# dusk-network/plonk

Measured on NVIDIA H100. Metric: proofs/sec @ 2^16 gates, higher is better.
Workload: dtype u32 limbs (Fr 256-bit / Fp 384-bit Montgomery)

## Files before the change

plonk_b200/csrc/prover.cu:

```cuda
#include <algorithm>
#include <mutex>
#include <vector>

#include "compress.h"
#include "internal.cuh"
#include "host_field.h"
#include "plonk_algebra.cuh"
#include "transcript.h"

namespace pb {

static std::atomic<int> g_force_throughput{0};

PB_D Fr ldg_fr(const uint4* p, size_t i) {
  uint4 a = __ldg(p + 2 * i), b = __ldg(p + 2 * i + 1);
  Fr r;
  r.v[0] = a.x; r.v[1] = a.y; r.v[2] = a.z; r.v[3] = a.w;
  r.v[4] = b.x; r.v[5] = b.y; r.v[6] = b.z; r.v[7] = b.w;
  return r;
}
PB_D Fr ld_fr_plain(const uint4* p, size_t i) {
  uint4 a = p[2 * i], b = p[2 * i + 1];
  Fr r;
  r.v[0] = a.x; r.v[1] = a.y; r.v[2] = a.z; r.v[3] = a.w;
// ... 209 lines not shown
  if (tid == 255 && totals) {
    Fr tot = lds_pair(sh[cur][255]);
    stg_fr(totals, blockIdx.x, tot);
  }
}

template <bool MUL, bool REV>
__global__ void k_scan_fixup(uint4* out, size_t n, const uint4* block_prefix) {
  const size_t i = (size_t)blockIdx.x * blockDim.x + threadIdx.x;
  if (i >= n) return;
  const size_t blk = i / 2048;
  if (blk == 0) return;
  const size_t j = REV ? (n - 1 - i) : i;
  stg_fr(out, j, scan_op<MUL>(ld_fr_plain(block_prefix, blk), ld_fr_plain(out, j)));
}

struct QuotArgs {
  const uint4* w8;
  const uint4* key8;
  const uint4* linear8;
  const uint4* l1_8;
  uint4* out;
  size_t n8;
  Fr alpha, beta, gamma, alpha_sq;
  SepPowers<Fr> ch_range, ch_logic, ch_fixed, ch_var;
  Fr edwards_d;
  Fr vh_inv[8];
  int has_range, has_logic, has_fixed, has_var;
};

__device__ __noinline__ Fr fr_mul_outlined(Fr a, Fr b) { return a * b; }

struct Q {
  Fr v;
  PB_D Q() {}
  PB_D Q(const Fr& f) : v(f) {}
  static PB_D Q one() { return Q(Fr::one()); }
  static PB_D Q zero() { return Q(Fr::zero()); }
  friend PB_D Q operator+(const Q& x, const Q& y) { return Q(x.v + y.v); }
  friend PB_D Q operator-(const Q& x, const Q& y) { return Q(x.v - y.v); }
  friend PB_D Q operator*(const Q& x, const Q& y) { return Q(fr_mul_outlined(x.v, y.v)); }
  PB_D Q sqr() const { return Q(fr_mul_outlined(v, v)); }
  PB_D Q dbl() const { return Q(v.dbl()); }
};

PB_D void quotient_point(const QuotArgs& q, size_t ws, size_t i, size_t iw, size_t ki, size_t oi) {
  const size_t n8 = q.n8;
  WireVals<Q> v;
  const Q z = ldg_fr(q.w8, i), z_w = ldg_fr(q.w8, iw);
  v.a = ldg_fr(q.w8, ws + i); v.a_w = ldg_fr(q.w8, ws + iw);
  v.b = ldg_fr(q.w8, 2 * ws + i); v.b_w = ldg_fr(q.w8, 2 * ws + iw);
  v.c = ldg_fr(q.w8, 3 * ws + i);
  v.d = ldg_fr(q.w8, 4 * ws + i); v.d_w = ldg_fr(q.w8, 4 * ws + iw);
  const Q pi = ldg_fr(q.w8, 5 * ws + i);
#define KEY(k) ldg_fr(q.key8, (size_t)(k) * n8 + ki)
  const Q q_l = KEY(Q_L), q_r = KEY(Q_R), q_c = KEY(Q_C);
  Q t = (v.a * v.b * KEY(Q_M) + v.a * q_l + v.b * q_r + v.c * KEY(Q_O) + v.d * KEY(Q_F) + q_c) * KEY(Q_ARITH);
  if (q.has_range) t = t + widget_range(q.ch_range, v) * KEY(Q_RANGE);
  if (q.has_logic) t = t + widget_logic(q.ch_logic, q_c, v) * KEY(Q_LOGIC);
  if (q.has_fixed) t = t + widget_fixed(q.ch_fixed, Q(q.edwards_d), q_l, q_r, q_c, v) * KEY(Q_FIXED);
  if (q.has_var) t = t + widget_var(q.ch_var, Q(q.edwards_d), v) * KEY(Q_VAR);
  t = t + pi;
  const Q x = ldg_fr(q.linear8, ki);
  const Q alpha = q.alpha, beta = q.beta, gamma = q.gamma;
  const Q bx = beta * x;
  Q ident = perm_ident(v, bx, gamma) * z * alpha;
  Q copy = perm_copy3(v, beta, gamma, [&](int j) { return Q(KEY(S1 + j)); }) * (v.d + beta * KEY(S4) + gamma) * z_w * alpha;
#undef KEY
  Q l1 = Q(ldg_fr(q.l1_8, ki)) * Q(q.alpha_sq);
  t = t + ident - copy + (z - Q::one()) * l1;
  stg_fr(q.out, oi, (t * Q(q.vh_inv[ki & 7])).v);
}

__global__ void __launch_bounds__(128) k_quotient(QuotArgs q) {
  const size_t i = (size_t)blockIdx.x * blockDim.x + threadIdx.x;
  if (i >= q.n8) return;
  quotient_point(q, q.n8, i, (i + 8) & (q.n8 - 1), i, i);
}
template <int MINB>
__global__ void __launch_bounds__(128, MINB) k_quotient_4n(QuotArgs q) {
  const size_t i = (size_t)blockIdx.x * blockDim.x + threadIdx.x;
  const size_t n4 = q.n8 >> 1;
  if (i >= n4) return;
  quotient_point(q, n4, i, (i + 4) & (n4 - 1), 2 * i, i);
}
__global__ void __launch_bounds__(128) k_quotient_pts(QuotArgs q) {
  const size_t k = threadIdx.x;
  if (k >= 8) return;
  quotient_point(q, 16, k, k + 8, 1 + (q.n8 >> 3) * k, k);
}

__global__ void k_any_nonzero(const uint4* p, size_t lo, size_t hi, unsigned* flag) {
  size_t i = lo + (size_t)blockIdx.x * blockDim.x + threadIdx.x;
  if (i >= hi) return;
  uint4 a = p[2 * i], b = p[2 * i + 1];
  if (a.x | a.y | a.z | a.w | b.x | b.y | b.z | b.w) atomicOr(flag, 1u);
}

__global__ void k_split_quotient(const uint4* t, size_t n, size_t n8, size_t stride, Fr b12, Fr b13, Fr b14, uint4* out) {
  size_t i = (size_t)blockIdx.x * blockDim.x + threadIdx.x;
  if (i >= stride) return;
  const unsigned k = blockIdx.y;
  Fr v = Fr::zero();
  if (k < 3) {
    if (i < n) v = ld_fr_plain(t, (size_t)k * n + i);
    if (i == n) v = (k == 0) ? b12 : (k == 1 ? b13 : b14);
    if (i == 0 && k == 1) v = v - b12;
    if (i == 0 && k == 2) v = v - b13;
  } else {
    if (3 * n + i < n8) v = ld_fr_plain(t, 3 * n + i);
    if (i == 0) v = v - b14;
  }
  stg_fr(out, (size_t)k * stride + i, v);
}

PB_D void cta_poly_eval(const uint4* poly, unsigned len, const Fr& x, uint4* out_slot) {
  __shared__ uint4 sh[256][2];
  const int tid = threadIdx.x;
  const size_t base = ((size_t)blockIdx.x * 256 + tid) * 8;
  Fr acc = Fr::zero();
  if (base < len) {
#pragma unroll
    for (int k = 7; k >= 0; k--) {
      const Fr c = (base + k < len) ? ld_fr_plain(poly, base + k) : Fr::zero();
      acc = acc * x + c;
    }
  }
  sh[tid][0] = make_uint4(acc.v[0], acc.v[1], acc.v[2], acc.v[3]);
  sh[tid][1] = make_uint4(acc.v[4], acc.v[5], acc.v[6], acc.v[7]);
  Fr pw = x.sqr().sqr().sqr();
  __syncthreads();
  for (int d = 1; d < 256; d <<= 1) {
    if ((tid & (2 * d - 1)) == 0) {
      const Fr v = lds_pair(sh[tid]) + lds_pair(sh[tid + d]) * pw;
      sh[tid][0] = make_uint4(v.v[0], v.v[1], v.v[2], v.v[3]);
      sh[tid][1] = make_uint4(v.v[4], v.v[5], v.v[6], v.v[7]);
      pw = pw.sqr();
    }
    __syncthreads();
  }
  if (tid == 0) stg_fr(out_slot, 0, lds_pair(sh[0]));
}

struct EvalJobs {
  const uint4* poly[16];
  unsigned len[16];
  Fr point[16];
  int njobs;
};
__global__ void __launch_bounds__(256) k_poly_eval(EvalJobs jobs, uint4* partial, unsigned nblocks) {
  const int j = blockIdx.y;
  cta_poly_eval(jobs.poly[j], jobs.len[j], jobs.point[j], partial + 2 * ((size_t)j * nblocks + blockIdx.x));
}
struct EvalRows {
  const uint4* base;
  size_t row_stride;
  unsigned len;
  Fr point[16];
};
__global__ void __launch_bounds__(256) k_poly_eval_rows(EvalRows jobs, uint4* partial, unsigned nblocks) {
  cta_poly_eval(jobs.base + 2 * (size_t)blockIdx.z * jobs.row_stride, jobs.len, jobs.point[blockIdx.y],
                partial + 2 * (((size_t)blockIdx.z * gridDim.y + blockIdx.y) * nblocks + blockIdx.x));
}
struct EvalPoints {
  Fr p[16];
};
__global__ void k_sum_rows(const uint4* partial, unsigned nblocks, EvalPoints pts, int npts, uint4* out) {
  const int j = blockIdx.x;
  if (threadIdx.x != 0) return;
  Fr step = pts.p[j % npts];
#pragma unroll 1
  for (int k = 0; k < 11; k++) step = step.sqr();
  Fr acc = Fr::zero();
#pragma unroll 1
  for (unsigned b = nblocks; b-- > 0;) acc = acc * step + ld_fr_plain(partial, (size_t)j * nblocks + b);
  stg_fr(out, j, acc);
}

struct Quot4nFix {
  Fr c;
  Fr g4n;
  Fr hinv8[8];
  Fr w8inv_pow[8];
};
__global__ void k_quot4n_fix(const uint4* tx, const uint4* ux, uint4* tcoef, size_t n4, Quot4nFix f, unsigned* flag) {
  const int j = threadIdx.x;
  if (j >= 8) return;
  Fr acc = Fr::zero();
  for (int k = 0; k < 8; k++) {
    const Fr e = (ld_fr_plain(tx, k) - ld_fr_plain(ux, k)) * f.c;
    acc = acc + e * f.w8inv_pow[(j * k) & 7];
  }
  const Fr t_hi = acc * f.hinv8[j];
  if (j == 7) {
    if (!t_hi.is_zero()) atomicOr(flag, 1u);
    return;
  }
  stg_fr(tcoef, j, ld_fr_plain(tcoef, j) - f.g4n * t_hi);
  stg_fr(tcoef, n4 + j, t_hi);
}

struct LinArgs {
  const uint4* poly[24];
  unsigned len[24];
  Fr coef[24];
  int nterms;
};
__global__ void k_lincomb(LinArgs a, size_t n, uint4* out) {
  size_t i = (size_t)blockIdx.x * blockDim.x + threadIdx.x;
  if (i >= n) return;
  Fr acc = Fr::zero();
  for (int k = 0; k < a.nterms; k++)
    if (i < a.len[k]) acc = acc + ld_fr_plain(a.poly[k], i) * a.coef[k];
  stg_fr(out, i, acc);
}

__global__ void k_mul_pointwise(const uint4* a, const uint4* b, size_t n, uint4* out) {
  size_t i = (size_t)blockIdx.x * blockDim.x + threadIdx.x;
  if (i < n) stg_fr(out, i, ld_fr_plain(a, i) * ld_fr_plain(b, i));
}
__global__ void k_sub_one(uint4* p, size_t n) {
  size_t i = (size_t)blockIdx.x * blockDim.x + threadIdx.x;
  if (i < n) stg_fr(p, i, ld_fr_plain(p, i) - Fr::one());
}
struct Period8 {
  Fr c[8];
};
__global__ void k_scale_period8(uint4* p, size_t n, Period8 c) {
  size_t i = (size_t)blockIdx.x * blockDim.x + threadIdx.x;
  if (i < n) stg_fr(p, i, ld_fr_plain(p, i) * c.c[i & 7]);
}

struct Quot4nConsts {
  Fr xs[16];
  Quot4nFix fix;
};

}

using pbh::HFr;

struct pb200_prover {
  std::vector<uint8_t> label;
  size_t constraints = 0, n = 0, n8 = 0;
  int log_n = 0;
  pb200_srs* srs = nullptr;
  pb200_srs* srs_lag = nullptr;
  uint32_t* d_wires = nullptr;
  uint4* d_polys = nullptr;
  uint4* d_key8 = nullptr;
  uint4* d_linear8 = nullptr;
  uint4* d_l1_8 = nullptr;
  uint4* d_sigma = nullptr;
  HFr vh_inv[8];
  pb::Fr edwards_d;
  pb::Quot4nConsts q4;
  int has_widget[4] = {0, 0, 0, 0};
  uint8_t comm[pb::N_POLY][48];
  size_t n_witnesses = 0;
  unsigned long long* d_labels = nullptr;
  size_t n_labels = 0;
  mutable std::mutex ws_mu;
  mutable std::vector<pb::Arena> ws_free;
  mutable std::vector<char*> ws_all;
  size_t ws_bytes = 0;
  mutable std::atomic<int> active{0};
};

namespace pb {

static Fr to_dev(const HFr& x) {
  Fr r;
  memcpy(r.v, x.v, 32);
  return r;
}
static HFr to_host(const Fr& x) {
  HFr r;
  memcpy(r.v, x.v, 32);
  return r;
}

template <bool MUL, bool REV>
static int fr_scan(const uint4* in, size_t n, uint4* out, cudaStream_t st, Arena* ar) {
  const unsigned nblk = div_up(n, 2048);
  uint4 *tot = nullptr, *tot_scan = nullptr;
  ScratchScope scope(ar, st);
  PB_ALLOC(scope, tot, (size_t)nblk * 32);
  PB_ALLOC(scope, tot_scan, (size_t)nblk * 32);
  PB_LAUNCH((k_scan_local<MUL, REV>), nblk, 256, 0, st, in, n, out, tot);
  if (nblk > 1) {
    PB_TRY((fr_scan<MUL, false>((const uint4*)tot, (size_t)nblk, tot_scan, st, ar)));
    PB_LAUNCH((k_scan_fixup<MUL, REV>), div_up(n, 256), 256, 0, st, out, n, (const uint4*)tot_scan);
  }
  PB_CUDA(cudaGetLastError());
  return 0;
}
static size_t fr_scan_bytes(size_t n) {
  const size_t nblk = div_up(n, 2048);
  return 2 * Arena::round_up(nblk * 32) + (nblk > 1 ? fr_scan_bytes(nblk) : 0);
}

enum ProofBuf { kWv, kZp, kNum, kDen, kW8, kQuot, kTcoef, kTq, kAgg, kPw, kScratch, kEvals, kPartial, kFlag, kProofBufs };
static void proof_buffers(size_t n, size_t bytes[kProofBufs]) {
  const size_t stride = n + 8;
  bytes[kWv] = 5 * n * 32;
  bytes[kZp] = 6 * stride * 32;
  bytes[kNum] = bytes[kDen] = n * 32;
  bytes[kW8] = 6 * 8 * n * 32;
  bytes[kQuot] = bytes[kTcoef] = 8 * n * 32;
  bytes[kTq] = 4 * stride * 32;
  bytes[kAgg] = bytes[kPw] = bytes[kScratch] = 2 * stride * 32;
  bytes[kEvals] = 16 * 32;
  bytes[kPartial] = (size_t)16 * div_up(stride, 2048) * 32;
  bytes[kFlag] = 4;
}

static void compress_affine(const uint64_t* raw, uint8_t out[48]) { pbh::g1_compress_raw(raw, out); }

void prover_free(pb200_prover* P);

struct PoolBlock {
  void* p = nullptr;
  cudaStream_t st;
  explicit PoolBlock(cudaStream_t s) : st(s) {}
  ~PoolBlock() {
    if (p) cudaFreeAsync(p, st);
  }
  cudaError_t alloc(size_t bytes) { return cudaMallocAsync(&p, bytes, st); }
  PoolBlock(const PoolBlock&) = delete;
  PoolBlock& operator=(const PoolBlock&) = delete;
};

struct LoadedProverKey {
  const uint8_t* poly[N_POLY];
  size_t poly_len[N_POLY];
  uint8_t comm[N_POLY][48];
};

static int prover_build(pb200_prover* P, const uint8_t* label, size_t label_len, size_t constraints, const uint64_t* selectors,
                        const uint32_t* wires, size_t n_witnesses, const uint8_t* srs_raw, size_t n_srs, cudaStream_t st,
                        const LoadedProverKey* loaded = nullptr, const pbz::CompressedDescription* comp = nullptr) {
  P->label.assign(label, label + label_len);
  P->constraints = constraints;
  P->n_witnesses = n_witnesses;
  size_t n_trim = 1;
  while (n_trim < constraints + 6) n_trim <<= 1;
  size_t keep = n_trim + 6;
  if (keep + 1 > n_srs) return fail(PB200_ERR_DEGREE_TOO_LARGE, "public parameters too small for this circuit (TruncatedDegreeTooLarge)");
  size_t n = 1;
  int log_n = 0;
  while (n < constraints) {
    n <<= 1;
    log_n++;
  }
  P->n = n;
  P->n8 = 8 * n;
  P->log_n = log_n;
  if (log_n + 3 >= 32) return fail(PB200_ERR_INVALID_DOMAIN, "quotient domain too large");
  PB_TRY(srs_upload(srs_raw, keep + 1, &P->srs, 0));
  {
    static const bool lagrange_env = [] {
      const char* e = getenv("PB200_LAGRANGE");
      return !e || atoi(e) != 0;
    }();
    if (lagrange_env && n >= 2 && keep + 1 >= n + 2) {
      uint4* comb = nullptr;
      PB_CUDA(cudaMalloc((void**)&comb, (n + 4) * 96));
      const uint4* mono = srs_points(P->srs);
      int rc = lagrange_key_dev(mono, log_n, comb, st);
      const size_t idx[4] = {0, 1, n, n + 1};
      cudaError_t e = cudaSuccess;
      for (int k = 0; k < 4 && e == cudaSuccess; k++)
        e = cudaMemcpyAsync(comb + 6 * (n + k), mono + 6 * idx[k], 96, cudaMemcpyDeviceToDevice, st);
      if (e == cudaSuccess) e = cudaStreamSynchronize(st);
      int lag_c = std::min(12, msm_window_for(n + 4));
      if (const char* env = getenv("PB200_LAG_C")) lag_c = atoi(env);
      if (lag_c < 2 || lag_c > 20) lag_c = 0;
      if (rc == 0 && e == cudaSuccess) rc = srs_from_device(comb, n + 4, &P->srs_lag, lag_c);
      cudaFree(comb);
      PB_TRY(rc);
      PB_CUDA(e);
    }
  }
  const size_t n8 = P->n8;
  PB_CUDA(cudaMalloc((void**)&P->d_wires, 4 * constraints * 4));
  PB_CUDA(cudaMalloc((void**)&P->d_polys, (size_t)N_POLY * n * 32));
  PB_CUDA(cudaMalloc((void**)&P->d_key8, (size_t)N_POLY * n8 * 32));
  PB_CUDA(cudaMalloc((void**)&P->d_linear8, n8 * 32));
  PB_CUDA(cudaMalloc((void**)&P->d_l1_8, n8 * 32));
  PB_CUDA(cudaMalloc((void**)&P->d_sigma, 4 * n * 32));
  PB_CUDA(cudaMemcpyAsync(P->d_wires, wires, 4 * constraints * 4, cudaMemcpyHostToDevice, st));

  if (loaded) {
    for (size_t g = 0; g < constraints; g++)
      for (int k = 0; k < 4; k++)
        if (wires[(size_t)k * constraints + g] >= n_witnesses) return fail(PB200_ERR_INVALID_ARG, "wire index out of range");
    PB_CUDA(cudaMemsetAsync(P->d_polys, 0, (size_t)N_POLY * n * 32, st));
    for (int k = 0; k < N_POLY; k++)
      if (loaded->poly_len[k])
        PB_CUDA(cudaMemcpyAsync(P->d_polys + 2 * (size_t)k * n, loaded->poly[k], loaded->poly_len[k] * 32, cudaMemcpyHostToDevice, st));
    PoolBlock flag_block(st);
    PB_CUDA(flag_block.alloc(4));
    unsigned* d_flag = (unsigned*)flag_block.p;
    PB_CUDA(cudaMemsetAsync(d_flag, 0, 4, st));
    PB_LAUNCH(k_fr_from_canonical, div_up((size_t)N_POLY * n, 256), 256, 0, st, P->d_polys, (size_t)N_POLY * n, d_flag);
    unsigned h_flag = 0;
    PB_CUDA(cudaMemcpyAsync(&h_flag, d_flag, 4, cudaMemcpyDeviceToHost, st));
    PB_CUDA(cudaStreamSynchronize(st));
    if (h_flag) return fail(PB200_ERR_POINT_MALFORMED, "InvalidData: a prover-key scalar is not canonical");
    memcpy(P->comm, loaded->comm, sizeof P->comm);
    const int widget_sel[4] = {Q_RANGE, Q_LOGIC, Q_FIXED, Q_VAR};
    for (int w = 0; w < 4; w++) P->has_widget[w] = (P->comm[widget_sel[w]][0] & 0x40) ? 0 : 1;
  } else {
    PoolBlock cols_block(st);
    PB_CUDA(cols_block.alloc((size_t)N_POLY * n * 32));
    uint4* cols = (uint4*)cols_block.p;
    if (!comp) {
      PB_CUDA(cudaMemsetAsync(cols, 0, (size_t)N_POLY * n * 32, st));
      PB_CUDA(cudaMemcpy2DAsync(cols, n * 32, selectors, constraints * 32, constraints * 32, 11, cudaMemcpyHostToDevice, st));
    } else {
      const size_t n_sc = comp->scalars.size() / 32, n_pw = comp->polynomials.size();
      PoolBlock tab_block(st);
      PB_CUDA(tab_block.alloc(Arena::round_up(n_sc * 32) + Arena::round_up(n_pw * 4) + constraints * 4 + 4));
      uint4* d_sc = (uint4*)tab_block.p;
      uint32_t* d_pw = (uint32_t*)((char*)tab_block.p + Arena::round_up(n_sc * 32));
      uint32_t* d_gp = d_pw + Arena::round_up(n_pw * 4) / 4;
      unsigned* d_flag = d_gp + constraints;
      PB_CUDA(cudaMemcpyAsync(d_sc, comp->scalars.data(), n_sc * 32, cudaMemcpyHostToDevice, st));
      PB_CUDA(cudaMemcpyAsync(d_pw, comp->polynomials.data(), n_pw * 4, cudaMemcpyHostToDevice, st));
      PB_CUDA(cudaMemcpyAsync(d_gp, comp->gate_poly.data(), constraints * 4, cudaMemcpyHostToDevice, st));
      PB_CUDA(cudaMemsetAsync(d_flag, 0, 4, st));
      PB_LAUNCH(k_fr_from_canonical, div_up(n_sc, 256), 256, 0, st, d_sc, n_sc, d_flag);
      PB_LAUNCH(k_expand_selectors, dim3(div_up(n, 256), pbz::kSelectors), 256, 0, st, (const uint4*)d_sc, (const uint32_t*)d_pw,
                (const uint32_t*)d_gp, constraints, n, cols);
      unsigned h_flag = 0;
      PB_CUDA(cudaMemcpyAsync(&h_flag, d_flag, 4, cudaMemcpyDeviceToHost, st));
      PB_CUDA(cudaStreamSynchronize(st));
      if (h_flag) return fail(PB200_ERR_SCALAR_MALFORMED, "BlsScalarMalformed: a compressed circuit's scalar is not canonical");
      PB_CUDA(cudaMalloc((void**)&P->d_labels, comp->labels.size() * 8));
      PB_CUDA(cudaMemcpy(P->d_labels, comp->labels.data(), comp->labels.size() * 8, cudaMemcpyHostToDevice));
      P->n_labels = comp->labels.size();
    }
    {
      const size_t n_ids = comp ? comp->labels.size() : n_witnesses;
      std::vector<std::vector<uint64_t>> wmap(n_ids);
      for (size_t g = 0; g < constraints; g++)
        for (int k = 0; k < 4; k++) {
          const uint32_t w = wires[(size_t)k * constraints + g];
          if (w >= n_ids) {
            return fail(PB200_ERR_INVALID_ARG, "wire index out of range");
          }
          wmap[w].push_back(((uint64_t)k << 40) | g);
        }
      std::vector<unsigned long long> sig(4 * n);
      for (int k = 0; k < 4; k++)
        for (size_t i = 0; i < n; i++) sig[(size_t)k * n + i] = ((uint64_t)k << 40) | i;
      for (auto& lst : wmap)
        for (size_t i = 0; i < lst.size(); i++) {
          const uint64_t cur = lst[i], nxt = lst[(i + 1) % lst.size()];
          sig[(size_t)(cur >> 40) * n + (cur & 0xffffffffffull)] = nxt;
        }
      PoolBlock sig_block(st);
      PB_CUDA(sig_block.alloc(4 * n * 8));
      unsigned long long* d_sig = (unsigned long long*)sig_block.p;
      PB_CUDA(cudaMemcpyAsync(d_sig, sig.data(), 4 * n * 8, cudaMemcpyHostToDevice, st));
      const uint4* w_half = nullptr;
      PB_TRY(get_twiddles(log_n, false, st, &w_half));
      PB_LAUNCH(k_sigma_lagrange, div_up(4 * n, 256), 256, 0, st, d_sig, n, w_half, cols + 2 * (size_t)S1 * n);
      PB_CUDA(cudaStreamSynchronize(st));
    }
    PB_TRY(ntt_run((const uint64_t*)cols, n, (uint64_t*)P->d_polys, log_n, 1, 0, N_POLY, n, n, st, nullptr));
    {
      std::vector<uint64_t> aff((size_t)N_POLY * 12);
      PB_TRY(msm_run(P->srs, 0, (const uint64_t*)P->d_polys, n, N_POLY, n, kMsmLatency, aff.data(), st, nullptr));
      for (int k = 0; k < N_POLY; k++) compress_affine(aff.data() + 12 * k, P->comm[k]);
      const int widget_sel[4] = {Q_RANGE, Q_LOGIC, Q_FIXED, Q_VAR};
      for (int w = 0; w < 4; w++) P->has_widget[w] = (P->comm[widget_sel[w]][0] & 0x40) ? 0 : 1;
    }
  }
  PB_TRY(ntt_run((const uint64_t*)P->d_polys, n, (uint64_t*)P->d_key8, log_n + 3, 0, 1, N_POLY, n, n8, st, nullptr));
  {
    HFr lin[2] = {HFr::zero(), HFr::one()};
    PoolBlock lin_block(st);
    PB_CUDA(lin_block.alloc(64));
    uint4* d_lin = (uint4*)lin_block.p;
    PB_CUDA(cudaMemcpyAsync(d_lin, lin, 64, cudaMemcpyHostToDevice, st));
    PB_TRY(ntt_run((const uint64_t*)d_lin, 2, (uint64_t*)P->d_linear8, log_n + 3, 0, 1, 1, 2, n8, st, nullptr));
    PB_CUDA(cudaStreamSynchronize(st));
  }
  {
    const HFr g = to_host(ntt_coset_gen(false)), w8n = to_host(ntt_group_gen(log_n + 3, false));
    HFr point = g.pow_u64(n), step = w8n.pow_u64(n);
    const HFr psi = to_host(ntt_size_inv(log_n + 3)) * HFr::from_u64(8);
    Period8 c;
    for (int i = 0; i < 8; i++) {
      const HFr vh = point - HFr::one();
      P->vh_inv[i] = vh.inv();
      c.c[i] = to_dev(vh * psi);
      point = point * step;
    }
    PB_CUDA(cudaMemcpyAsync(P->d_l1_8, P->d_linear8, n8 * 32, cudaMemcpyDeviceToDevice, st));
    PB_LAUNCH(k_sub_one, div_up(n8, 256), 256, 0, st, P->d_l1_8, n8);
    PB_LAUNCH(k_batch_div, div_up(div_up(n8, 8), 128), 128, 0, st, (const uint4*)nullptr, (const uint4*)P->d_l1_8, n8, P->d_l1_8);
    PB_LAUNCH(k_scale_period8, div_up(n8, 256), 256, 0, st, P->d_l1_8, n8, c);
  }
  {
    P->edwards_d = to_dev(pbh::edwards_d());
    const HFr g = to_host(ntt_coset_gen(false)), w8n = to_host(ntt_group_gen(log_n + 3, false));
    const HFr h = g * w8n, w8r = w8n.pow_u64(n), wn = to_host(ntt_group_gen(log_n, false)), g4n = g.pow_u64(4 * n);
    HFr xs[16];
    xs[0] = h;
    for (int k = 1; k < 8; k++) xs[k] = xs[k - 1] * w8r;
    for (int k = 0; k < 8; k++) xs[8 + k] = xs[k] * wn;
    for (int k = 0; k < 16; k++) P->q4.xs[k] = to_dev(xs[k]);
    P->q4.fix.c = to_dev((g4n.dbl().neg()).inv());
    P->q4.fix.g4n = to_dev(g4n);
    const HFr h_inv = h.inv(), w8i = w8r.inv();
    HFr hj = HFr::from_u64(8).inv(), wp = HFr::one();
    for (int j = 0; j < 8; j++) {
      P->q4.fix.hinv8[j] = to_dev(hj);
      P->q4.fix.w8inv_pow[j] = to_dev(wp);
      hj = hj * h_inv;
      wp = wp * w8i;
    }
  }
  PB_TRY(ntt_run((const uint64_t*)(P->d_polys + 2 * (size_t)S1 * n), n, (uint64_t*)P->d_sigma, log_n, 0, 0, 4, n, n, st, nullptr));
  PB_CUDA(cudaGetLastError());
  PB_CUDA(cudaStreamSynchronize(st));
  {
    const size_t stride = n + 8;
    size_t call = std::max((size_t)6 * n8 * 32, fr_scan_bytes(stride));
    call = std::max(call, msm_workspace_bytes(P->srs, std::min(stride, srs_len(P->srs)), 4));
    if (P->srs_lag) call = std::max(call, msm_workspace_bytes(P->srs_lag, n + 4, 4));
    size_t bytes[kProofBufs];
    proof_buffers(n, bytes);
    P->ws_bytes = call;
    for (size_t b : bytes) P->ws_bytes += Arena::round_up(b);
    P->ws_bytes += Arena::round_up(P->n_labels * 32);
  }
  return 0;
}

int prover_new(const uint8_t* label, size_t label_len, size_t constraints, const uint64_t* selectors,
               const uint32_t* wires, size_t n_witnesses, const uint8_t* srs_raw, size_t n_srs, pb200_prover** out) {
  if (constraints == 0) return fail(PB200_ERR_INVALID_ARG, "empty circuit");
  pb200_prover* P = new pb200_prover();
  const int rc = prover_build(P, label, label_len, constraints, selectors, wires, n_witnesses, srs_raw, n_srs, thread_stream());
  if (rc != 0) {
    prover_free(P);
    return rc;
  }
  *out = P;
  return 0;
}

int prover_from_compressed(const uint8_t* label, size_t label_len, const uint8_t* bytes, size_t len, const uint8_t* srs_raw,
                           size_t n_srs, pb200_prover** out) {
  pbz::CompressedDescription d;
  PB_TRY(pbz::decode(bytes, len, n_srs, &d));
  if (d.gates() == 0) return fail(PB200_ERR_INVALID_ARG, "empty circuit");
  pb200_prover* P = new pb200_prover();
  const int rc = prover_build(P, label, label_len, d.gates(), nullptr, d.wires.data(), (size_t)d.witnesses, srs_raw, n_srs,
                              thread_stream(), nullptr, &d);
  if (rc != 0) {
    prover_free(P);
    return rc;
  }
  *out = P;
  return 0;
}

int prover_from_bytes(const uint8_t* bytes, size_t len, const uint32_t* wires, size_t n_witnesses, pb200_prover** out) {
  auto be64 = [](const uint8_t* p) {
    uint64_t v = 0;
    for (int i = 0; i < 8; i++) v = (v << 8) | p[i];
    return v;
  };
  auto le64 = [](const uint8_t* p) {
    uint64_t v = 0;
    for (int i = 7; i >= 0; i--) v = (v << 8) | p[i];
    return v;
  };
  const int short_rc = PB200_ERR_INVALID_ARG, bad_rc = PB200_ERR_POINT_MALFORMED;
  if (len < 48) return fail(short_rc, "NotEnoughBytes: serialized prover shorter than its header");
  const uint64_t label_len = be64(bytes), pk_len = be64(bytes + 8), ck_len = be64(bytes + 16), vk_len = be64(bytes + 24),
                 size = be64(bytes + 32), constraints = be64(bytes + 40);
  const uint8_t* p = bytes + 48;
  size_t left = len - 48;
  if (label_len > left || pk_len > left - label_len || ck_len > left - label_len - pk_len || vk_len > left - label_len - pk_len - ck_len)
    return fail(short_rc, "NotEnoughBytes: serialized prover shorter than its sections");
  size_t pow2 = 1;
  while (pow2 < constraints) pow2 <<= 1;
  if (constraints == 0 || pow2 != size) return fail(bad_rc, "InvalidData: size is not the next power of two of the constraint count");
  const uint8_t* label = p;
  const uint8_t* pk = label + label_len;
  const uint8_t* ck = pk + pk_len;
  const uint8_t* vk = ck + ck_len;
  LoadedProverKey key;
  {
    size_t off = 0;
    auto need = [&](size_t k) { return k <= pk_len - off; };
    if (pk_len < 16) return fail(short_rc, "NotEnoughBytes: prover key");
    const uint64_t n = le64(pk), eval_size = le64(pk + 8);
    off = 16;
    if (n != size) return fail(bad_rc, "InvalidData: prover key domain differs from the prover's size");
    if (eval_size != 8 * n * 32 + 172) return fail(bad_rc, "InvalidData: evaluations are not over the 8n domain");
    for (int i = 0; i < N_POLY; i++) {
      if (!need(8)) return fail(short_rc, "NotEnoughBytes: prover key polynomial header");
      const uint64_t cnt = le64(pk + off);
      off += 8;
      if (cnt > n) return fail(bad_rc, "InvalidData: polynomial longer than the domain");
      if (!need(cnt * 32)) return fail(short_rc, "NotEnoughBytes: prover key polynomial");
      key.poly[kKeyFileOrder[i]] = pk + off;
      key.poly_len[kKeyFileOrder[i]] = (size_t)cnt;
      off += cnt * 32;
      if (!need(eval_size)) return fail(short_rc, "NotEnoughBytes: prover key evaluations");
      off += eval_size;
    }
    if (!need(2 * eval_size)) return fail(short_rc, "NotEnoughBytes: linear / vanishing evaluations");
  }
  if (vk_len < 8 + 15 * 48) return fail(short_rc, "NotEnoughBytes: verifier key");
  for (int i = 0; i < N_POLY; i++) memcpy(key.comm[kKeyFileOrder[i]], vk + 8 + 48 * i, 48);
  size_t n_pts = 0;
  PB_TRY(raw_commit_key_parse(ck, ck_len, 1, &n_pts, nullptr));
  std::vector<uint8_t> raw(n_pts * 96);
  PB_TRY(raw_commit_key_parse(ck, ck_len, 1, &n_pts, raw.data()));
  PB_TRY(g1_check_raw(raw.data(), n_pts));
  pb200_prover* P = new pb200_prover();
  const int rc = prover_build(P, label, label_len, constraints, nullptr, wires, n_witnesses, raw.data(), n_pts, thread_stream(), &key);
  if (rc != 0) {
    prover_free(P);
    return rc;
  }
  *out = P;
  return 0;
}

struct KeyStreamer {
  static constexpr size_t kChunk = (size_t)8 << 20;
  cudaStream_t st;
  uint4* d_buf[2] = {nullptr, nullptr};
  uint8_t* h_buf[2] = {nullptr, nullptr};
  cudaEvent_t ev[2] = {nullptr, nullptr};
  struct Pending {
    uint8_t* dst = nullptr;
    size_t count = 0;
    bool points = false;
  } pend[2];
  unsigned issued = 0;

  explicit KeyStreamer(cudaStream_t s) : st(s) {}
  ~KeyStreamer() {
    for (int b = 0; b < 2; b++) {
      if (pend[b].count) cudaEventSynchronize(ev[b]);
      if (d_buf[b]) cudaFreeAsync(d_buf[b], st);
      if (ev[b]) cudaEventDestroy(ev[b]);
    }
  }
  KeyStreamer(const KeyStreamer&) = delete;
  KeyStreamer& operator=(const KeyStreamer&) = delete;

  int init() {
    for (int b = 0; b < 2; b++) {
      PB_CUDA(cudaMallocAsync((void**)&d_buf[b], kChunk, st));
      h_buf[b] = (uint8_t*)pinned_scratch(kChunk, b);
      if (!h_buf[b]) return fail(PB200_ERR_CUDA, "pinned staging buffer allocation failed");
      PB_CUDA(cudaEventCreateWithFlags(&ev[b], cudaEventBlockingSync | cudaEventDisableTiming));
// ... 190 lines not shown
  PB_TRY(get_twiddles(log_n, false, st, &w_half));

  Arena arena;
  {
    std::lock_guard<std::mutex> lk(P->ws_mu);
    if (!P->ws_free.empty()) {
      arena = P->ws_free.back();
      P->ws_free.pop_back();
    }
  }
  if (!arena.base) {
    char* mem = nullptr;
    PB_CUDA(cudaMalloc((void**)&mem, P->ws_bytes));
    arena.base = mem;
    arena.size = P->ws_bytes;
    std::lock_guard<std::mutex> lk(P->ws_mu);
    P->ws_all.push_back(mem);
  }
  arena.off = 0;
  struct Release {
    const pb200_prover* P;
    Arena* a;
    cudaStream_t st;
    ~Release() {
      stream_wait(st);
      a->off = 0;
      std::lock_guard<std::mutex> lk(P->ws_mu);
      P->ws_free.push_back(*a);
    }
  } release{P, &arena, st};
  Arena* ar = &arena;
  ScratchScope scope(ar, st);
  const unsigned eval_blocks = div_up(stride, 2048);
  size_t bytes[kProofBufs];
  void* kept[kProofBufs];
  proof_buffers(n, bytes);
  for (int i = 0; i < kProofBufs; i++) PB_ALLOC(scope, kept[i], bytes[i]);
  uint4 *wv = (uint4*)kept[kWv], *zp = (uint4*)kept[kZp], *num = (uint4*)kept[kNum], *den = (uint4*)kept[kDen], *w8 = (uint4*)kept[kW8],
        *quot = (uint4*)kept[kQuot], *tcoef = (uint4*)kept[kTcoef], *tq = (uint4*)kept[kTq], *agg = (uint4*)kept[kAgg],
        *pw = (uint4*)kept[kPw], *scratch = (uint4*)kept[kScratch], *evals_d = (uint4*)kept[kEvals], *partial = (uint4*)kept[kPartial];
  unsigned* flag = (unsigned*)kept[kFlag];
  uint4 *wp = zp + 2 * stride, *pi_dense = wv + 2 * 4 * n;

  uint64_t aff[4 * 12];
  uint8_t c48[N_COMM][48];
  Challenges ch;

  if (P->d_labels) {
    uint4* dense = nullptr;
    PB_ALLOC(scope, dense, P->n_labels * 32);
    PB_LAUNCH(k_gather_witnesses, div_up(P->n_labels, 256), 256, 0, st, (const uint4*)d_wit, (const unsigned long long*)P->d_labels,
              P->n_labels, dense);
    d_wit = (const uint64_t*)dense;
  }

  PB_LAUNCH(k_gather_wires, dim3(div_up(n, 256), 4), 256, 0, st, (const uint4*)d_wit, (const uint32_t*)P->d_wires, P->constraints, n, wv);
  if (n_pi) {
    PB_CUDA(cudaMemsetAsync(pi_dense, 0, n * 32, st));
    for (size_t i = 0; i < n_pi; i++)
      PB_CUDA(cudaMemcpyAsync(pi_dense + 2 * pi_idx[i], PIV + i, 32, cudaMemcpyHostToDevice, st));
  }
  PB_CUDA(cudaMemsetAsync(zp, 0, 6 * stride * 32, st));
  PB_TRY(ntt_run((const uint64_t*)wv, n, (uint64_t*)wp, log_n, 1, 0, n_pi ? 5 : 4, n, stride, st, ar));
  {
    BlindArgs ba;
    ba.nb = 2;
    ba.npoly = 4;
    for (int p = 0; p < 4; p++)
      for (int i = 0; i < 2; i++) ba.b[p][i] = to_dev(BL[2 * p + i]);
    PB_LAUNCH(k_blind, 1, 32, 0, st, wp, stride, n, ba);
  }
  if (P->srs_lag) {
    uint4* sc = w8;
    PB_CUDA(cudaMemcpy2DAsync(sc, stride * 32, wv, n * 32, n * 32, 4, cudaMemcpyDeviceToDevice, st));
    BlindArgs ba;
    ba.nb = 2;
    ba.npoly = 4;
    for (int p = 0; p < 4; p++)
      for (int i = 0; i < 2; i++) ba.b[p][i] = to_dev(BL[2 * p + i]);
    PB_LAUNCH(k_lagrange_tail, 1, 32, 0, st, sc, stride, n, ba);
    PB_TRY(msm_run(P->srs_lag, 0, (const uint64_t*)sc, n + 4, 4, stride, MsmShape{true, busy()}, aff, st, ar));
  } else {
    PB_TRY(msm_run(P->srs, 0, (const uint64_t*)wp, n + 2, 4, stride, dense_shape(), aff, st, ar));
  }
  for (int k = 0; k < 4; k++) compress_affine(aff + 12 * k, c48[C_A + k]);

  pbh::challenge_beta_gamma(tr, c48[0], ch);
  const HFr beta = ch.beta, gamma = ch.gamma;
  PB_LAUNCH(k_perm_terms, div_up(n, 128), 128, 0, st, (const uint4*)wv, (const uint4*)P->d_sigma, w_half, n, to_dev(beta), to_dev(gamma), num, den);
  PB_LAUNCH(k_batch_div, div_up(div_up(n, 8), 128), 128, 0, st, (const uint4*)num, (const uint4*)den, n, num);
  PB_TRY((fr_scan<true, false>(num, n, den, st, ar)));
  PB_TRY(ntt_run((const uint64_t*)den, n, (uint64_t*)zp, log_n, 1, 0, 1, n, stride, st, ar));
  {
    BlindArgs ba;
    ba.nb = 3;
    ba.npoly = 1;
    for (int i = 0; i < 3; i++) ba.b[0][i] = to_dev(BL[8 + i]);
    PB_LAUNCH(k_blind, 1, 32, 0, st, zp, stride, n, ba);
  }
  PB_TRY(msm_run(P->srs, 0, (const uint64_t*)zp, n + 3, 1, stride, dense_shape(), aff, st, ar));
  compress_affine(aff, c48[C_Z]);

  pbh::challenge_alpha(tr, c48[0], ch);
  const HFr alpha = ch.alpha;
  static const bool quot4n_env = [] {
    const char* e = getenv("PB200_QUOT4N");
    return !e || atoi(e) != 0;
  }();
  const bool quot4n = quot4n_env && n >= 16;
  const size_t n4 = 4 * n;
  size_t t_len = n8;
  QuotArgs q;
  {
    q.w8 = w8; q.key8 = P->d_key8; q.linear8 = P->d_linear8; q.l1_8 = P->d_l1_8; q.out = quot; q.n8 = n8;
    q.alpha = to_dev(alpha); q.beta = to_dev(beta); q.gamma = to_dev(gamma); q.alpha_sq = to_dev(alpha.sqr());
    auto powers = [](const HFr& c) {
      const SepPowers<HFr> h = sep_powers(c);
      SepPowers<Fr> s;
      s.ch = to_dev(h.ch); s.k = to_dev(h.k); s.k2 = to_dev(h.k2); s.k3 = to_dev(h.k3); s.k4 = to_dev(h.k4);
      return s;
    };
    q.ch_range = powers(ch.range); q.ch_logic = powers(ch.logic); q.ch_fixed = powers(ch.fixed); q.ch_var = powers(ch.var);
    q.edwards_d = P->edwards_d;
    for (int i = 0; i < 8; i++) q.vh_inv[i] = to_dev(P->vh_inv[i]);
    q.has_range = P->has_widget[0]; q.has_logic = P->has_widget[1]; q.has_fixed = P->has_widget[2]; q.has_var = P->has_widget[3];
  }
  unsigned char* stage = (unsigned char*)pinned_scratch(1024, 1);
  if (!stage) return fail(PB200_ERR_CUDA, "pinned staging buffer");
  volatile unsigned& h_flag = *(volatile unsigned*)(stage + 512);
  if (!quot4n) {
    PB_TRY(ntt_run((const uint64_t*)zp, n + 3, (uint64_t*)w8, log_n + 3, 0, 1, n_pi ? 6 : 5, stride, n8, st, ar));
    if (!n_pi) PB_CUDA(cudaMemsetAsync(w8 + 2 * 5 * n8, 0, n8 * 32, st));
    PB_LAUNCH(k_quotient, div_up(n8, 128), 128, 0, st, q);
    PB_TRY(ntt_run((const uint64_t*)quot, n8, (uint64_t*)tcoef, log_n + 3, 1, 1, 1, n8, n8, st, ar));
    PB_CUDA(cudaMemsetAsync(flag, 0, 4, st));
    PB_LAUNCH(k_any_nonzero, div_up(n8 - 7 * n, 256), 256, 0, st, (const uint4*)tcoef, 7 * n, n8, flag);
    PB_CUDA(cudaMemcpyAsync(stage + 512, flag, 4, cudaMemcpyDeviceToHost, st));
  } else {
    PB_TRY(ntt_run((const uint64_t*)zp, n + 3, (uint64_t*)w8, log_n + 2, 0, 1, n_pi ? 6 : 5, stride, n4, st, ar));
    if (!n_pi) PB_CUDA(cudaMemsetAsync(w8 + 2 * 5 * n4, 0, n4 * 32, st));
    static const int quot_occ = [] {
      const char* e = getenv("PB200_QUOT_OCC");
      return e ? atoi(e) : 3;
    }();
    if (quot_occ == 3)
      PB_LAUNCH(k_quotient_4n<3>, div_up(n4, 128), 128, 0, st, q);
    else
      PB_LAUNCH(k_quotient_4n<2>, div_up(n4, 128), 128, 0, st, q);
    PB_TRY(ntt_run((const uint64_t*)quot, n4, (uint64_t*)tcoef, log_n + 2, 1, 1, 1, n4, n4, st, ar));
    uint4* wpts = w8 + 2 * 6 * n4;
    uint4* tx = wpts + 2 * 96;
    uint4* ux = tx + 2 * 8;
    uint4* part4 = ux + 2 * 8;
    const unsigned blocks4 = div_up(n4, 2048);
    const Quot4nConsts& qc = P->q4;
    const int rows = n_pi ? 6 : 5;
    {
      EvalRows er;
      er.base = zp; er.row_stride = stride; er.len = (unsigned)n + 3;
      for (int j = 0; j < 16; j++) er.point[j] = qc.xs[j];
      EvalPoints ep;
      for (int j = 0; j < 16; j++) ep.p[j] = qc.xs[j];
      PB_LAUNCH(k_poly_eval_rows, dim3(eval_blocks, 16, rows), 256, 0, st, er, part4, eval_blocks);
      PB_LAUNCH(k_sum_rows, 16 * rows, 32, 0, st, (const uint4*)part4, eval_blocks, ep, 16, wpts);
    }
    if (!n_pi) PB_CUDA(cudaMemsetAsync(wpts + 2 * 16 * 5, 0, 16 * 32, st));
    QuotArgs qp = q;
    qp.w8 = wpts;
    qp.out = tx;
    PB_LAUNCH(k_quotient_pts, 1, 128, 0, st, qp);
    {
      EvalRows er;
      er.base = tcoef; er.row_stride = 0; er.len = (unsigned)n4;
      for (int j = 0; j < 16; j++) er.point[j] = qc.xs[j];
      EvalPoints ep;
      for (int j = 0; j < 16; j++) ep.p[j] = qc.xs[j];
      PB_LAUNCH(k_poly_eval_rows, dim3(blocks4, 8, 1), 256, 0, st, er, part4, blocks4);
      PB_LAUNCH(k_sum_rows, 8, 32, 0, st, (const uint4*)part4, blocks4, ep, 16, ux);
    }
    PB_CUDA(cudaMemsetAsync(flag, 0, 4, st));
    PB_LAUNCH(k_quot4n_fix, 1, 32, 0, st, (const uint4*)tx, (const uint4*)ux, tcoef, n4, qc.fix, flag);
    PB_CUDA(cudaMemcpyAsync(stage + 512, flag, 4, cudaMemcpyDeviceToHost, st));
    t_len = n4 + 7;
  }
  PB_LAUNCH(k_split_quotient, dim3(div_up(stride, 256), 4), 256, 0, st, (const uint4*)tcoef, n, t_len, stride, to_dev(BL[11]), to_dev(BL[12]), to_dev(BL[13]), tq);
  const size_t key_len = srs_len(P->srs);
  const size_t tlen = std::min(stride, key_len);
  PB_TRY(msm_run(P->srs, 0, (const uint64_t*)tq, tlen, 4, stride, dense_shape(), aff, st, ar));
  if (h_flag) return fail(PB200_ERR_UNSATISFIED, "CircuitUnsatisfied");
  for (int k = 0; k < 4; k++) compress_affine(aff + 12 * k, c48[C_T_LOW + k]);

  pbh::challenge_z(tr, c48[0], ch);
  const HFr z_ch = ch.z;
  const HFr zw = z_ch * to_host(ntt_group_gen(log_n, false));
  HFr ev[N_EVAL];
  {
    EvalJobs jobs;
    jobs.njobs = 15;
    auto poly = [&](int k) { return (const uint4*)(P->d_polys + 2 * (size_t)k * n); };
    const uint4* ps[15] = {wp, wp + 2 * stride, wp + 4 * stride, wp + 6 * stride, wp, wp + 2 * stride, wp + 6 * stride,
                           poly(Q_ARITH), poly(Q_C), poly(Q_L), poly(Q_R), poly(S1), poly(S2), poly(S3), zp};
    const unsigned ls[15] = {(unsigned)n + 2, (unsigned)n + 2, (unsigned)n + 2, (unsigned)n + 2, (unsigned)n + 2, (unsigned)n + 2, (unsigned)n + 2,
                             (unsigned)n, (unsigned)n, (unsigned)n, (unsigned)n, (unsigned)n, (unsigned)n, (unsigned)n, (unsigned)n + 3};
    const bool shifted[15] = {0, 0, 0, 0, 1, 1, 1, 0, 0, 0, 0, 0, 0, 0, 1};
    for (int j = 0; j < 15; j++) {
      jobs.poly[j] = ps[j];
      jobs.len[j] = ls[j];
      jobs.point[j] = to_dev(shifted[j] ? zw : z_ch);
    }
    EvalPoints ep;
    for (int j = 0; j < 15; j++) ep.p[j] = jobs.point[j];
    ep.p[15] = Fr::zero();
    PB_LAUNCH(k_poly_eval, dim3(eval_blocks, 15), 256, 0, st, jobs, partial, eval_blocks);
    PB_LAUNCH(k_sum_rows, 15, 32, 0, st, (const uint4*)partial, eval_blocks, ep, 16, evals_d);
    PB_CUDA(cudaMemcpyAsync(stage, evals_d, 15 * 32, cudaMemcpyDeviceToHost, st));
    PB_CUDA(stream_wait(st));
    memcpy(ev, stage, 15 * 32);
  }
  pbh::challenge_v(tr, ev, ch);
  const HFr v = ch.v, v_w = ch.v_w;
  {
    const HFr z_n = z_ch.pow_u64(n);
    const HFr l1_z = (z_n - HFr::one()) * to_host(ntt_size_inv(log_n)) * (z_ch - HFr::one()).inv();
    const LinScalars ls = linearisation_scalars(ev, ch, z_n, l1_z);
    HFr vp[12];
    vp[0] = HFr::one();
    for (int i = 1; i < 12; i++) vp[i] = vp[i - 1] * v;
    HFr sel[N_POLY];
    for (int k = 0; k < N_POLY; k++) sel[k] = ls.sel[k];
    sel[Q_ARITH] = sel[Q_ARITH] + vp[8];
    sel[Q_C] = sel[Q_C] + vp[9];
    sel[Q_L] = sel[Q_L] + vp[10];
    sel[Q_R] = sel[Q_R] + vp[11];
    auto poly = [&](int k) { return (const uint4*)(P->d_polys + 2 * (size_t)k * n); };
    LinArgs la;
    int t = 0;
    auto term = [&](const uint4* p, size_t len, const HFr& coef) { la.poly[t] = p; la.len[t] = (unsigned)len; la.coef[t] = to_dev(coef); t++; };
    for (int k = Q_M; k <= Q_VAR; k++) term(poly(k), n, sel[k]);
    term(zp, n + 3, ls.z);
    term(poly(S4), n, sel[S4]);
    for (int j = 0; j < 4; j++) term(tq + 2 * j * stride, stride, ls.t[j]);
    term(wp, n + 2, vp[1]);
    term(wp + 2 * stride, n + 2, vp[2]);
    term(wp + 4 * stride, n + 2, vp[3]);
    term(wp + 6 * stride, n + 2, vp[4]);
    term(poly(S1), n, vp[5]);
    term(poly(S2), n, vp[6]);
    term(poly(S3), n, vp[7]);
    la.nterms = t;
    PB_LAUNCH(k_lincomb, div_up(stride, 128), 128, 0, st, la, stride, agg);
    LinArgs lb;
    t = 0;
    auto term2 = [&](const uint4* p, size_t len, const HFr& coef) { lb.poly[t] = p; lb.len[t] = (unsigned)len; lb.coef[t] = to_dev(coef); t++; };
    term2(zp, n + 3, HFr::one());
    term2(wp, n + 2, v_w);
    term2(wp + 2 * stride, n + 2, v_w.sqr());
    term2(wp + 6 * stride, n + 2, v_w.sqr() * v_w);
    lb.nterms = t;
    PB_LAUNCH(k_lincomb, div_up(stride, 128), 128, 0, st, lb, stride, agg + 2 * stride);
    const HFr pts[2] = {z_ch, zw};
    for (int w = 0; w < 2; w++) {
      uint4* c_w = agg + 2 * (size_t)w * stride;
      uint4* pw_w = pw + 2 * (size_t)w * stride;
      uint4* sc_w = scratch + 2 * (size_t)w * stride;
      PB_TRY(fill_powers(pw_w, stride, to_dev(pts[w]), Fr::one(), st));
      PB_LAUNCH(k_mul_pointwise, div_up(stride, 128), 128, 0, st, (const uint4*)c_w, (const uint4*)pw_w, stride, sc_w);
      PB_TRY((fr_scan<false, true>(sc_w, stride, c_w, st, ar)));
      const HFr zi = pts[w].inv();
      PB_TRY(fill_powers(pw_w, stride, to_dev(zi), to_dev(zi), st));
      PB_LAUNCH(k_mul_pointwise, div_up(stride, 128), 128, 0, st, (const uint4*)c_w, (const uint4*)pw_w, stride, c_w);
    }
    const size_t wlen = std::min(stride, key_len);
    PB_TRY(msm_run(P->srs, 0, (const uint64_t*)agg, wlen, 2, stride, dense_shape(), aff, st, ar));
    compress_affine(aff, c48[C_W_Z]);
    compress_affine(aff + 12, c48[C_W_ZW]);
  }
  memcpy(out_proof, c48, sizeof c48);
  for (int i = 0; i < N_EVAL; i++) {
    HFr cnon = ev[i].from_mont();
    memcpy(out_proof + kProofEvalAt + 32 * i, cnon.v, 32);
  }
  return 0;
}

static int unsatisfied_columns(const uint4* sel, const uint4* d_wit, const uint32_t* d_wires, size_t constraints, size_t n,
                               const uint64_t* pi_idx, const uint64_t* pi_vals, size_t n_pi, size_t cap, uint64_t* rows,
                               int32_t* families, size_t* n_unsatisfied, cudaStream_t st) {
  ScratchScope scope(nullptr, st);
  uint4* wv = nullptr;
  PB_ALLOC(scope, wv, (n_pi ? 5 : 4) * n * 32);
  PB_LAUNCH(k_gather_wires, dim3(div_up(n, 256), 4), 256, 0, st, d_wit, d_wires, constraints, n, wv);
  uint4* pi_dense = nullptr;
  if (n_pi) {
    pi_dense = wv + 2 * 4 * n;
    PB_CUDA(cudaMemsetAsync(pi_dense, 0, n * 32, st));
    for (size_t i = 0; i < n_pi; i++)
      PB_CUDA(cudaMemcpyAsync(pi_dense + 2 * pi_idx[i], pi_vals + 4 * i, 32, cudaMemcpyHostToDevice, st));
  }
  return unsatisfied_run(sel, wv, pi_dense, n, constraints, cap, rows, families, n_unsatisfied, st);
}

}

using namespace pb;

extern "C" {

int pb200_prover_new(const uint8_t* label, size_t label_len, size_t n_constraints, const uint64_t* selectors,
                     const uint32_t* wires, size_t n_witnesses, const uint8_t* srs_raw, size_t n_srs_points,
                     pb200_prover_t** out) {
  PB_TRY(ensure_init());
  if (!selectors || !wires || !srs_raw || !out) return fail(PB200_ERR_INVALID_ARG, "null argument");
  return prover_new(label, label_len, n_constraints, selectors, wires, n_witnesses, srs_raw, n_srs_points, out);
}

int pb200_prover_from_compressed(const uint8_t* label, size_t label_len, const uint8_t* bytes, size_t len,
                                 const uint8_t* srs_raw, size_t n_srs_points, pb200_prover_t** out) {
  if ((!label && label_len) || !bytes || !srs_raw || !out) return fail(PB200_ERR_INVALID_ARG, "null argument");
  PB_TRY(ensure_init());
  return prover_from_compressed(label, label_len, bytes, len, srs_raw, n_srs_points, out);
}

int pb200_throughput_mode(int on) {
  g_force_throughput.store(on ? 1 : 0, std::memory_order_relaxed);
  return 0;
}

int pb200_prover_from_bytes(const uint8_t* bytes, size_t len, const uint32_t* wires, size_t n_witnesses, pb200_prover_t** out) {
  PB_TRY(ensure_init());
  if (!bytes || !wires || !out) return fail(PB200_ERR_INVALID_ARG, "null argument");
  return prover_from_bytes(bytes, len, wires, n_witnesses, out);
}
// ... 118 lines not shown
```

Before: 204.6.

## Evaluate polynomials on 8-point coset via decimation instead of per-point Horner

Replaces the separate per-point Horner evaluations (16 points per row, plus 8 points on the quotient) with one coset-structured kernel. It splits each polynomial into 8 residue classes, evaluates each class at y^8 once, and recombines them with a small size-8 DFT using powers of the 8th roots. This removes about eightfold redundant field multiplications and coefficient reads, and it merges the row and tail evaluations into one eval launch and one sum launch. It relies on the evaluation points forming cosets of the 8th roots of unity, and it adds more complex reduction and indexing logic.

```diff
diff --git a/plonk_b200/csrc/prover.cu b/plonk_b200/csrc/prover.cu
--- a/plonk_b200/csrc/prover.cu
+++ b/plonk_b200/csrc/prover.cu
@@ -385,16 +385,6 @@
   const int j = blockIdx.y;
   cta_poly_eval(jobs.poly[j], jobs.len[j], jobs.point[j], partial + 2 * ((size_t)j * nblocks + blockIdx.x));
 }
-struct EvalRows {
-  const uint4* base;
-  size_t row_stride;
-  unsigned len;
-  Fr point[16];
-};
-__global__ void __launch_bounds__(256) k_poly_eval_rows(EvalRows jobs, uint4* partial, unsigned nblocks) {
-  cta_poly_eval(jobs.base + 2 * (size_t)blockIdx.z * jobs.row_stride, jobs.len, jobs.point[blockIdx.y],
-                partial + 2 * (((size_t)blockIdx.z * gridDim.y + blockIdx.y) * nblocks + blockIdx.x));
-}
 struct EvalPoints {
   Fr p[16];
 };
@@ -410,6 +400,126 @@
   stg_fr(out, j, acc);
 }
 
+struct Coset8Consts {
+  Fr spow[2][8];
+  Fr ypow[2][16];
+  Fr w8pow[8];
+};
+constexpr unsigned kC8Per = 4;
+constexpr unsigned kC8Block = 256 * kC8Per;
+struct Coset8Jobs {
+  const uint4* rows;
+  size_t row_stride;
+  unsigned row_len, row_blocks;
+  int nrows;
+  const uint4* tail;
+  unsigned tail_len, tail_blocks;
+};
+PB_D Fr shfl_xor_fr(const Fr& a, int m) {
+  Fr r;
+#pragma unroll
+  for (int i = 0; i < 8; i++) r.v[i] = __shfl_xor_sync(0xffffffffu, a.v[i], m);
+  return r;
+}
+PB_D void sts_pair(uint4* s, const Fr& a) {
+  s[0] = make_uint4(a.v[0], a.v[1], a.v[2], a.v[3]);
+  s[1] = make_uint4(a.v[4], a.v[5], a.v[6], a.v[7]);
+}
+__global__ void __launch_bounds__(256) k_coset8_eval(Coset8Jobs J, Coset8Consts C, uint4* partial) {
+  __shared__ uint4 sh[8][8][2];
+  const unsigned nrow_blk = 2 * J.nrows * J.row_blocks;
+  const uint4* poly;
+  unsigned len, b, nb;
+  int cs;
+  if (blockIdx.x < nrow_blk) {
+    const unsigned job = blockIdx.x / J.row_blocks;
+    b = blockIdx.x - job * J.row_blocks;
+    poly = J.rows + 2 * (size_t)(job >> 1) * J.row_stride;
+    len = J.row_len; nb = J.row_blocks; cs = job & 1;
+  } else {
+    b = blockIdx.x - nrow_blk;
+    poly = J.tail; len = J.tail_len; nb = J.tail_blocks; cs = 0;
+  }
+  const unsigned tid = threadIdx.x, lane = tid & 31, warp = tid >> 5;
+  const size_t groups = (len + 7) / 8;
+  const size_t end = (b + 1 == nb) ? groups : (size_t)(b + 1) * kC8Block;
+  const size_t g0 = (size_t)b * kC8Block + tid;
+  const int top = g0 < end ? (int)((end - 1 - g0) / 256) : -1;
+  auto coef = [&](int i, int r) {
+    const size_t k = 8 * (g0 + 256 * (size_t)i) + r;
+    return k < len ? ld_fr_plain(poly, k) : Fr::zero();
+  };
+  Fr acc[8];
+#pragma unroll
+  for (int r = 0; r < 8; r++) acc[r] = top >= 0 ? coef(top, r) : Fr::zero();
+  const Fr step = C.ypow[cs][8];
+#pragma unroll 1
+  for (int i = top - 1; i >= 0; i--)
+#pragma unroll
+    for (int r = 0; r < 8; r++) acc[r] = acc[r] * step + coef(i, r);
+  Fr w = Fr::one();
+#pragma unroll
+  for (int k = 0; k < 5; k++)
+    if (lane >> k & 1) w = w * C.ypow[cs][k];
+#pragma unroll
+  for (int r = 0; r < 8; r++) {
+    Fr v = acc[r] * w;
+#pragma unroll
+    for (int m = 16; m > 0; m >>= 1) v = v + shfl_xor_fr(v, m);
+    if (lane == 0) sts_pair(sh[warp][r], v);
+  }
+  __syncthreads();
+  if (tid < 64) {
+    Fr v = lds_pair(sh[tid >> 3][tid & 7]);
+#pragma unroll
+    for (int k = 0; k < 3; k++)
+      if (tid >> (3 + k) & 1) v = v * C.ypow[cs][5 + k];
+    sts_pair(sh[tid >> 3][tid & 7], v);
+  }
+  __syncthreads();
+  if (tid < 8) {
+    Fr s = lds_pair(sh[0][tid]);
+#pragma unroll
+    for (int k = 1; k < 8; k++) s = s + lds_pair(sh[k][tid]);
+    stg_fr(partial, 8 * (size_t)blockIdx.x + tid, s);
+  }
+}
+__global__ void __launch_bounds__(256) k_coset8_sum(Coset8Jobs J, Coset8Consts C, const uint4* partial, uint4* wpts, uint4* ux) {
+  __shared__ uint4 sh[8][8][2];
+  const unsigned job = blockIdx.x, nrj = 2 * J.nrows;
+  const unsigned nb = job < nrj ? J.row_blocks : J.tail_blocks;
+  const int cs = job < nrj ? (job & 1) : 0;
+  const unsigned tid = threadIdx.x, r = tid & 7, p = tid >> 3;
+  Fr w = Fr::one();
+#pragma unroll
+  for (int k = 0; k < 5; k++)
+    if (p >> k & 1) w = w * C.ypow[cs][10 + k];
+  Fr acc = Fr::zero();
+#pragma unroll 1
+  for (unsigned b = p; b < nb; b += 32) {
+    acc = acc + ld_fr_plain(partial, 8 * ((size_t)job * J.row_blocks + b) + r) * w;
+    w = w * C.ypow[cs][15];
+  }
+  acc = acc + shfl_xor_fr(acc, 8);
+  acc = acc + shfl_xor_fr(acc, 16);
+  if ((tid & 31) < 8) sts_pair(sh[tid >> 5][r], acc);
+  __syncthreads();
+  if (tid < 8) {
+    Fr f = lds_pair(sh[0][r]);
+#pragma unroll
+    for (int k = 1; k < 8; k++) f = f + lds_pair(sh[k][r]);
+    sts_pair(sh[0][r], f * C.spow[cs][r]);
+  }
+  __syncthreads();
+  if (tid < 8) {
+    Fr out = lds_pair(sh[0][0]);
+#pragma unroll
+    for (int j = 1; j < 8; j++) out = out + lds_pair(sh[0][j]) * C.w8pow[(j * tid) & 7];
+    if (job < nrj) stg_fr(wpts, 16 * (job >> 1) + 8 * (job & 1) + tid, out);
+    else stg_fr(ux, tid, out);
+  }
+}
+
 struct Quot4nFix {
   Fr c;
   Fr g4n;
@@ -465,7 +575,7 @@
 }
 
 struct Quot4nConsts {
-  Fr xs[16];
+  Coset8Consts c8;
   Quot4nFix fix;
 };
 
@@ -741,11 +851,14 @@
     P->edwards_d = to_dev(pbh::edwards_d());
     const HFr g = to_host(ntt_coset_gen(false)), w8n = to_host(ntt_group_gen(log_n + 3, false));
     const HFr h = g * w8n, w8r = w8n.pow_u64(n), wn = to_host(ntt_group_gen(log_n, false)), g4n = g.pow_u64(4 * n);
-    HFr xs[16];
-    xs[0] = h;
-    for (int k = 1; k < 8; k++) xs[k] = xs[k - 1] * w8r;
-    for (int k = 0; k < 8; k++) xs[8 + k] = xs[k] * wn;
-    for (int k = 0; k < 16; k++) P->q4.xs[k] = to_dev(xs[k]);
+    const HFr shift[2] = {h, h * wn};
+    for (int c = 0; c < 2; c++) {
+      HFr p = HFr::one();
+      for (int r = 0; r < 8; r++, p = p * shift[c]) P->q4.c8.spow[c][r] = to_dev(p);
+      for (int i = 0; i < 16; i++, p = p.sqr()) P->q4.c8.ypow[c][i] = to_dev(p);
+    }
+    HFr w8k = HFr::one();
+    for (int k = 0; k < 8; k++, w8k = w8k * w8r) P->q4.c8.w8pow[k] = to_dev(w8k);
     P->q4.fix.c = to_dev((g4n.dbl().neg()).inv());
     P->q4.fix.g4n = to_dev(g4n);
     const HFr h_inv = h.inv(), w8i = w8r.inv();
@@ -1242,32 +1355,22 @@
     uint4* tx = wpts + 2 * 96;
     uint4* ux = tx + 2 * 8;
     uint4* part4 = ux + 2 * 8;
-    const unsigned blocks4 = div_up(n4, 2048);
     const Quot4nConsts& qc = P->q4;
     const int rows = n_pi ? 6 : 5;
     {
-      EvalRows er;
-      er.base = zp; er.row_stride = stride; er.len = (unsigned)n + 3;
-      for (int j = 0; j < 16; j++) er.point[j] = qc.xs[j];
-      EvalPoints ep;
-      for (int j = 0; j < 16; j++) ep.p[j] = qc.xs[j];
-      PB_LAUNCH(k_poly_eval_rows, dim3(eval_blocks, 16, rows), 256, 0, st, er, part4, eval_blocks);
-      PB_LAUNCH(k_sum_rows, 16 * rows, 32, 0, st, (const uint4*)part4, eval_blocks, ep, 16, wpts);
+      Coset8Jobs cj;
+      cj.rows = zp; cj.row_stride = stride; cj.row_len = (unsigned)n + 3; cj.nrows = rows;
+      cj.row_blocks = (unsigned)std::max<size_t>(1, div_up(n + 3, 8) / kC8Block);
+      cj.tail = tcoef; cj.tail_len = (unsigned)n4;
+      cj.tail_blocks = (unsigned)std::max<size_t>(1, (n4 / 8) / kC8Block);
+      PB_LAUNCH(k_coset8_eval, 2 * rows * cj.row_blocks + cj.tail_blocks, 256, 0, st, cj, qc.c8, part4);
+      PB_LAUNCH(k_coset8_sum, 2 * rows + 1, 256, 0, st, cj, qc.c8, (const uint4*)part4, wpts, ux);
     }
     if (!n_pi) PB_CUDA(cudaMemsetAsync(wpts + 2 * 16 * 5, 0, 16 * 32, st));
     QuotArgs qp = q;
     qp.w8 = wpts;
     qp.out = tx;
     PB_LAUNCH(k_quotient_pts, 1, 128, 0, st, qp);
-    {
-      EvalRows er;
-      er.base = tcoef; er.row_stride = 0; er.len = (unsigned)n4;
-      for (int j = 0; j < 16; j++) er.point[j] = qc.xs[j];
-      EvalPoints ep;
-      for (int j = 0; j < 16; j++) ep.p[j] = qc.xs[j];
-      PB_LAUNCH(k_poly_eval_rows, dim3(blocks4, 8, 1), 256, 0, st, er, part4, blocks4);
-      PB_LAUNCH(k_sum_rows, 8, 32, 0, st, (const uint4*)part4, blocks4, ep, 16, ux);
-    }
     PB_CUDA(cudaMemsetAsync(flag, 0, 4, st));
     PB_LAUNCH(k_quot4n_fix, 1, 32, 0, st, (const uint4*)tx, (const uint4*)ux, tcoef, n4, qc.fix, flag);
     PB_CUDA(cudaMemcpyAsync(stage + 512, flag, 4, cudaMemcpyDeviceToHost, st));
```

Result: faster. 217.6 (median of 6 runs) (+6.4%).
